# krispy-kenay/WebDGS

Hardware: AMD Instinct MI355X
Metric: training iters/sec (fwd+bwd+Adam), 1M Gaussians @1080p SH3 (higher is better)
Workload: dtype f32

## Files before the change

### webdgs_amd/csrc/common.h

```cpp
#pragma once
#include <hip/hip_runtime.h>

#include <cstdint>
#include <cstdio>
#include <map>
#include <string>
#include <vector>

#include "../../include/webdgs.h"
#include "devmem.h"

typedef uint32_t u32;
typedef int32_t i32;

void wdgs_set_error(const char* fmt, ...);

#define WDGS_CHECK_HIP(expr)                                                                      \
    do {                                                                                          \
        hipError_t _e = (expr);                                                                   \
        if (_e != hipSuccess) {                                                                   \
            wdgs_set_error("%s failed: %s (%s:%d)", #expr, hipGetErrorString(_e), __FILE__, __LINE__); \
            return WDGS_E_HIP;                                                                    \
        }                                                                                         \
    } while (0)

#define WDGS_REQUIRE(cond, code, ...)  \
    do {                               \
        if (!(cond)) {                 \
            wdgs_set_error(__VA_ARGS__); \
            return (code);             \
        }                              \
    } while (0)

#define WDGS_TRY(expr)                 \
    do {                               \
        int _r = (expr);               \
        if (_r != WDGS_OK) return _r;  \
    } while (0)

struct wdgs_device {
    int ordinal = 0;
    hipStream_t stream = nullptr;
    bool own_stream = false;
    hipStream_t lanes[WDGS_MAX_LANES] = {};
    hipEvent_t lane_events[WDGS_MAX_LANES] = {};
    hipEvent_t lane_marks[WDGS_MAX_BATCH_VIEWS] = {};
    int lane = 0;
    hipEvent_t ticket_events[WDGS_TICKET_RING] = {};
    uint64_t ticket_next = 1;
    u32* host_guard = nullptr;
    bool profiling = false;
    bool capturing = false;
    struct Pending { const char* name; hipEvent_t a, b; };
    std::vector<Pending> pending;
    std::vector<hipEvent_t> event_pool;
    struct Total { u32 launches = 0; float ms = 0.f; };
    std::map<std::string, Total> totals;
    std::vector<wdgs_tiled_forward*> forwards;
    std::map<const void*, wdgs_tiled_forward*> range_tables;
    std::vector<wdgs_tiled_forward*> capture_consumes;
    std::vector<void*> dead_command_buffers;
    int num_cus = 256;
    double* ssim_partials = nullptr;
    u32 ssim_partials_count = 0;
};

inline hipError_t wdgs_sync_lanes(wdgs_device* d) {
    for (int l = 1; l < WDGS_MAX_LANES; l++) {
        if (!d->lanes[l]) continue;
        const hipError_t e = hipStreamSynchronize(d->lanes[l]);
        if (e != hipSuccess) return e;
    }
    return hipStreamSynchronize(d->lanes[0] ? d->lanes[0] : d->stream);
}

struct KernelScope {
    wdgs_device* d;
    const char* name;
    hipEvent_t a = nullptr, b = nullptr;
    KernelScope(wdgs_device* dev, const char* n) : d(dev), name(n) {
        if (d->profiling && !d->capturing) {
            a = take(); b = take();
            (void)hipEventRecord(a, d->stream);
        }
    }
    ~KernelScope() {
        if (a) {
            (void)hipEventRecord(b, d->stream);
            d->pending.push_back({name, a, b});
        }
    }
    hipEvent_t take() {
        if (!d->event_pool.empty()) { hipEvent_t e = d->event_pool.back(); d->event_pool.pop_back(); return e; }
        hipEvent_t e; (void)hipEventCreate(&e); return e;
    }
};

#define WDGS_LAUNCH(dev, kname, kernel, grid, block, shmem, ...)                           \
    do {                                                                                   \
        KernelScope _ks((dev), (kname));                                                   \
        hipLaunchKernelGGL(kernel, (grid), (block), (shmem), (dev)->stream, __VA_ARGS__);  \
    } while (0)

constexpr u32 CS_PLANES = 7;
struct CsView {
    float4* planes;
    u32 pitch;
    __device__ __forceinline__ float4& quad(u32 k, u32 idx) const { return planes[(size_t)k * pitch + idx]; }
};

__device__ __forceinline__ u32 xcd_contiguous(u32 b, u32 g) {
    const u32 k = b & 7u, j = b >> 3, q = g >> 3, r = g & 7u;
    return k * q + min(k, r) + j;
}

static inline u32 ceil_div(u32 a, u32 b) { return (a + b - 1u) / b; }
static inline u32 bits_for(u32 v) {
    u32 b = 0;
    while (v) { b++; v >>= 1; }
    return b;
}

constexpr u32 SSIM_WG_PER_CU = 2;
static inline size_t align_up(size_t a, size_t b) { return (a + b - 1) / b * b; }

using wdgs::DevMem;
bool wdgs_device_alive(const wdgs_device* d);

struct RenderSettings { float gaussian_scaling, sh_deg, viewport_x, viewport_y, point_size_px, gaussian_mode, max_splat_radius_px; };
struct TileInfo { u32 num_tiles_x, num_tiles_y, total_tiles, max_tile_entries; };
```

### webdgs_amd/csrc/project.hip

```cpp
#include "launch.h"
#include "wgslm.h"

namespace {

__constant__ float SH_C2c[5] = {1.0925484305920792f, -1.0925484305920792f, 0.31539156525252005f, -1.0925484305920792f, 0.5462742152960396f};
__constant__ float SH_C3c[7] = {-0.5900435899266435f, 2.890611442640554f, -0.4570457994644658f, 0.3731763325901154f,
                                -0.4570457994644658f, 1.445305721320277f, -0.5900435899266435f};

struct ShRow { u32 w[24]; };
WD_DEV ShRow load_sh_row(const u32* __restrict__ sh_buffer, u32 idx, u32 sh_deg) {
    ShRow r;
#pragma unroll
    for (u32 i = 0; i < 24u; i++) r.w[i] = 0u;
    const uint4* q = reinterpret_cast<const uint4*>(sh_buffer + (size_t)idx * 24);
    const u32 nq = (sh_deg == 0u) ? 1u : (sh_deg == 1u) ? 2u : (sh_deg == 2u) ? 4u : 6u;
#pragma unroll
    for (u32 i = 0; i < 6u; i++)
        if (i < nq) { const uint4 v = q[i]; r.w[4 * i] = v.x; r.w[4 * i + 1] = v.y; r.w[4 * i + 2] = v.z; r.w[4 * i + 3] = v.w; }
    return r;
}
WD_DEV float sh_half(const ShRow& sh, u32 h) {
    const u32 w = sh.w[h >> 1];
    return (h & 1u) ? wd_unpack_hi(w) : wd_unpack_lo(w);
}
// ... 241 lines not shown
            if (total > capacity) host_mirror[2] = total;
            host_mirror[3] = 0u;
        }
    }
}

__global__ __launch_bounds__(256) void emit_kernel(u32 n, const u32* __restrict__ splats, const u32* __restrict__ depths,
                                                    const u32* __restrict__ tile_counts, u32* __restrict__ tile_offsets,
                                                    const u32* __restrict__ block_offsets, RenderSettings settings, TileInfo ti,
                                                    u32* __restrict__ keys, u32* __restrict__ values, u32 capacity) {
    __shared__ u32 s_pre[4][64], s_org[4][64], s_w[4][64], s_inv[4][64], s_dep[4][64];
    __shared__ u32 s_wtot[4];
    const u32 idx = blockIdx.x * blockDim.x + threadIdx.x;
    const u32 lane = threadIdx.x & 63u, wave = threadIdx.x >> 6;
    u32 cnt = 0u, org = 0u, width = 1u, depth16 = 0u;
    if (idx < n) {
        const u32 num_tiles = tile_counts[idx];
        if (num_tiles != 0u) {
            const uint2 w01 = *reinterpret_cast<const uint2*>(splats + (size_t)idx * 6);
            const vec2 ndc = V2(wd_unpack_lo(w01.x), wd_unpack_hi(w01.x));
            const float cap = (settings.max_splat_radius_px > 0.0f) ? settings.max_splat_radius_px : 1e9f;
            const vec2 ext = V2(wd_min(wd_unpack_lo(w01.y), cap), wd_min(wd_unpack_hi(w01.y), cap));
            const vec2 viewport = V2(settings.viewport_x, settings.viewport_y);
            const TileBox tb = tile_box(ndc, ext, viewport, ti.num_tiles_x, ti.num_tiles_y, false);
            if (tb.valid) {
                width = tb.max_x - tb.min_x + 1u;
                cnt = width * (tb.max_y - tb.min_y + 1u);
                org = tb.min_y * ti.num_tiles_x + tb.min_x;
                depth16 = depths[idx] >> 16u;
            }
        }
    }
    u32 inc = cnt;
#pragma unroll
    for (u32 d = 1; d < 64; d <<= 1) {
        const u32 t = __shfl_up(inc, d, 64);
        if (lane >= d) inc += t;
    }
    const u32 total = (u32)__shfl((int)inc, 63, 64);
    const u32 wave_first = idx - lane;
    u32 start0;
    if (block_offsets) {
        if (lane == 0u) s_wtot[wave] = total;
        __syncthreads();
        start0 = block_offsets[blockIdx.x];
#pragma unroll
        for (u32 w = 0; w < 4u; w++) start0 += (w < wave) ? s_wtot[w] : 0u;
        if (idx < n) tile_offsets[idx] = start0 + inc - cnt;
        if (total == 0u) return;
    } else {
        if (total == 0u) return;
        start0 = tile_offsets[wave_first];
    }
    s_pre[wave][lane] = inc - cnt;
    s_org[wave][lane] = org;
    s_w[wave][lane] = width;
    s_inv[wave][lane] = 0xFFFFFFFFu / width + 1u;
    s_dep[wave][lane] = depth16;
    __builtin_amdgcn_fence(__ATOMIC_RELEASE, "wavefront");
    __builtin_amdgcn_wave_barrier();
    const u32* pre = s_pre[wave];
    for (u32 e = lane; e < total; e += 64u) {
        u32 o = 0u;
#pragma unroll
        for (u32 step = 32u; step >= 1u; step >>= 1) o += (pre[o + step] <= e) ? step : 0u;
        const u32 k = e - pre[o];
        const u32 w = s_w[wave][o];
        const u32 row = (w == 1u) ? k : __umulhi(k, s_inv[wave][o]);
        const u32 tile_id = s_org[wave][o] + row * ti.num_tiles_x + (k - row * w);
        const u32 key_idx = start0 + e;
        if (key_idx < capacity) {
            keys[key_idx] = ((tile_id + 1u) << 16u) | s_dep[wave][o];
            values[key_idx] = wave_first + o;
        }
    }
}


constexpr u32 ES_CHUNK = 2048;
constexpr u32 ES_ROUNDS = ES_CHUNK / 256;
__global__ __launch_bounds__(256) void emit_scatter_kernel(u32 n, const u32* __restrict__ splats, const u32* __restrict__ depths,
                                                            const u32* __restrict__ tile_counts, u32* __restrict__ tile_offsets,
                                                            const u32* __restrict__ block_offsets, RenderSettings settings, TileInfo ti,
                                                            const u32* __restrict__ column_offsets ,
                                                            const u32* __restrict__ column_totals, u32 inv_ntx ,
                                                            u32* __restrict__ keys, u32* __restrict__ values, u32 capacity) {
    __shared__ u32 s_pre[256];
    __shared__ u32 s_box[256];
    __shared__ u32 s_inv[256], s_dep[256];
    __shared__ u32 whist[4][256];
    __shared__ u32 s_gbase[256];
    __shared__ u32 s_delta[256];
    __shared__ __align__(16) u32 s_keys[ES_CHUNK];
    __shared__ __align__(16) u32 s_vals[ES_CHUNK];
    __shared__ u32 s_wsum[4], s_tsum[4];
    unsigned short* const s_own = reinterpret_cast<unsigned short*>(s_vals);
    const u32 wg = xcd_contiguous(blockIdx.x, gridDim.x);
    const u32 idx = wg * 256u + threadIdx.x;
    const u32 lane = threadIdx.x & 63u, wave = threadIdx.x >> 6;
    const u32 ntx = ti.num_tiles_x;
    u32 cnt = 0u, ox = 0u, oy = 0u, width = 1u, depth16 = 0u;
    const u32 col = threadIdx.x;
    const bool in_range = idx < n;
    const u32 num_tiles = in_range ? tile_counts[idx] : 0u;
    const uint2 w01 = in_range ? *reinterpret_cast<const uint2*>(splats + (size_t)idx * 6) : make_uint2(0u, 0u);
    const u32 depth_all = in_range ? depths[idx] : 0u;
    const u32 tot_c = (col < ntx) ? column_totals[col] : 0u;
    const u32 off_c = (col < ntx) ? column_offsets[(size_t)col * gridDim.x + wg] : 0u;
    const u32 wg_offset = block_offsets[wg];
    if (num_tiles != 0u) {
        const vec2 ndc = V2(wd_unpack_lo(w01.x), wd_unpack_hi(w01.x));
        const float cap = (settings.max_splat_radius_px > 0.0f) ? settings.max_splat_radius_px : 1e9f;
        const vec2 ext = V2(wd_min(wd_unpack_lo(w01.y), cap), wd_min(wd_unpack_hi(w01.y), cap));
        const vec2 viewport = V2(settings.viewport_x, settings.viewport_y);
        const TileBox tb = tile_box(ndc, ext, viewport, ti.num_tiles_x, ti.num_tiles_y, false);
        if (tb.valid) {
            width = tb.max_x - tb.min_x + 1u;
            cnt = width * (tb.max_y - tb.min_y + 1u);
            ox = tb.min_x; oy = tb.min_y;
            depth16 = depth_all >> 16u;
        }
    }
    u32 inc = cnt;
#pragma unroll
    for (u32 d = 1; d < 64; d <<= 1) {
        const u32 t = __shfl_up(inc, d, 64);
        if (lane >= d) inc += t;
    }
    if (lane == 63u) s_wsum[wave] = inc;
    u32 tinc = tot_c;
#pragma unroll
    for (u32 d = 1; d < 64; d <<= 1) {
        const u32 t = __shfl_up(tinc, d, 64);
        if (lane >= d) tinc += t;
    }
    if (lane == 63u) s_tsum[wave] = tinc;
    __syncthreads();
    u32 woff = 0u, total = 0u, tbase = tinc - tot_c;
#pragma unroll
    for (u32 w = 0; w < 4u; w++) {
        const u32 v = s_wsum[w];
        woff += (w < wave) ? v : 0u;
        total += v;
        tbase += (w < wave) ? s_tsum[w] : 0u;
    }
    const u32 pre = woff + inc - cnt;
    if (idx < n) tile_offsets[idx] = wg_offset + pre;
    if (total == 0u) return;
    s_pre[threadIdx.x] = pre;
    s_box[threadIdx.x] = ox | (oy << 8u) | (width << 16u);
    s_inv[threadIdx.x] = 0xFFFFFFFFu / width + 1u;
    s_dep[threadIdx.x] = depth16;
    s_gbase[col] = tbase + off_c;
    const unsigned long long lt_mask = (1ull << lane) - 1ull;
    const u32 wg_first = wg * 256u;
    auto column_of = [&](u32 key) { const u32 t = (key >> 16u) - 1u; return t - __umulhi(t, inv_ntx) * ntx; };
    for (u32 c0 = 0u; c0 < total; c0 += ES_CHUNK) {
        const u32 n_here = min(ES_CHUNK, total - c0);
        const u32 per_wave = ((n_here + 3u) / 4u + 63u) & ~63u;
        const u32 rounds = per_wave / 64u;
#pragma unroll
        for (u32 w = 0; w < 4u; w++) whist[w][threadIdx.x] = 0u;
        reinterpret_cast<uint4*>(s_own)[threadIdx.x] = make_uint4(0u, 0u, 0u, 0u);
        __syncthreads();
        if (cnt != 0u && pre + cnt > c0 && pre < c0 + n_here) s_own[max(pre, c0) - c0] = (unsigned short)(threadIdx.x + 1u);
        __syncthreads();
        {
            const uint4 q = reinterpret_cast<const uint4*>(s_own)[threadIdx.x];
            u32 o[8] = {q.x & 0xFFFFu, q.x >> 16, q.y & 0xFFFFu, q.y >> 16, q.z & 0xFFFFu, q.z >> 16, q.w & 0xFFFFu, q.w >> 16};
#pragma unroll
            for (u32 j = 1; j < 8u; j++) o[j] = max(o[j], o[j - 1u]);
            u32 minc = o[7];
#pragma unroll
            for (u32 d = 1; d < 64; d <<= 1) {
                const u32 t = __shfl_up(minc, d, 64);
                if (lane >= d) minc = max(minc, t);
            }
            if (lane == 63u) s_wsum[wave] = minc;
            __syncthreads();
            u32 carry = __shfl_up(minc, 1, 64);
            if (lane == 0u) carry = 0u;
#pragma unroll
            for (u32 w = 0; w < 4u; w++) carry = max(carry, (w < wave) ? s_wsum[w] : 0u);
#pragma unroll
            for (u32 j = 0; j < 8u; j++) o[j] = max(o[j], carry);
            reinterpret_cast<uint4*>(s_own)[threadIdx.x] = make_uint4(o[0] | (o[1] << 16), o[2] | (o[3] << 16), o[4] | (o[5] << 16), o[6] | (o[7] << 16));
        }
        __syncthreads();
        u32 kk[ES_ROUNDS], vv[ES_ROUNDS], rk[ES_ROUNDS];
#pragma unroll
        for (u32 j = 0; j < ES_ROUNDS; j++) {
            kk[j] = 0xFFFFFFFFu; vv[j] = 0u; rk[j] = 0u;
            if (j < rounds) {
                const u32 i = wave * per_wave + j * 64u + lane;
                const bool valid = i < n_here;
                const u32 o = valid ? (u32)s_own[i] - 1u : 0u;
                const u32 k = c0 + (valid ? i : 0u) - s_pre[o];
                const u32 box = s_box[o];
                const u32 w = box >> 16u;
                const u32 row = (w == 1u) ? k : __umulhi(k, s_inv[o]);
                const u32 cx = (box & 0xFFu) + (k - row * w);
                const u32 tile_id = (((box >> 8u) & 0xFFu) + row) * ntx + cx;
                kk[j] = valid ? (((tile_id + 1u) << 16u) | s_dep[o]) : 0xFFFFFFFFu;
                vv[j] = wg_first + o;
                const u32 digit = valid ? cx : 0u;
                unsigned long long m = __ballot(valid);
#pragma unroll
                for (u32 b = 0; b < 8; b++) {
                    const bool bit = (digit >> b) & 1u;
                    const unsigned long long bal = __ballot(bit);
                    m &= bit ? bal : ~bal;
                }
                const u32 pre_c = whist[wave][digit];
                const u32 below = (u32)__popcll(m & lt_mask);
                rk[j] = pre_c + below;
                if (valid && below == 0u) whist[wave][digit] = pre_c + (u32)__popcll(m);
            }
        }
        __syncthreads();
        {
            u32 cnt_c = 0u;
#pragma unroll
            for (u32 w = 0; w < 4u; w++) cnt_c += whist[w][col];
            u32 cinc = cnt_c;
#pragma unroll
            for (u32 d = 1; d < 64; d <<= 1) {
                const u32 t = __shfl_up(cinc, d, 64);
                if (lane >= d) cinc += t;
            }
            if (lane == 63u) s_wsum[wave] = cinc;
            __syncthreads();
            u32 lstart = cinc - cnt_c;
#pragma unroll
            for (u32 w = 0; w < 4u; w++) lstart += (w < wave) ? s_wsum[w] : 0u;
            const u32 gb = s_gbase[col];
            s_delta[col] = gb - lstart;
            s_gbase[col] = gb + cnt_c;
            u32 run = lstart;
#pragma unroll
            for (u32 w = 0; w < 4u; w++) {
                const u32 c = whist[w][col];
                whist[w][col] = run;
                run += c;
            }
        }
        __syncthreads();
#pragma unroll
        for (u32 j = 0; j < ES_ROUNDS; j++) {
            if (j < rounds) {
                const u32 i = wave * per_wave + j * 64u + lane;
                if (i < n_here) {
                    const u32 lpos = whist[wave][column_of(kk[j])] + rk[j];
                    s_keys[lpos] = kk[j];
                    s_vals[lpos] = vv[j];
                }
            }
        }
        __syncthreads();
        for (u32 e = threadIdx.x; e < n_here; e += 256u) {
            const u32 key = s_keys[e];
            const u32 pos = s_delta[column_of(key)] + e;
            if (pos < capacity) {
                keys[pos] = key;
                values[pos] = s_vals[e];
            }
        }
        __syncthreads();
    }
}

}

int launch_project_count(wdgs_device* dev, u32 n, const u32* gaussians, const u32* sh, const float* camera, const RenderSettings& st, const TileInfo& ti, u32* splats,
                         u32* depths, u32* counts, u32* visible_shards, u32* block_counts, u32* column_counts, const u32* dc_words, u32* nf_stamp, const u32* nf_frame) {
    if (n == 0) return WDGS_OK;
    WDGS_LAUNCH(dev, "project_count", project_count_kernel, dim3(ceil_div(n, 256)), dim3(256), 0, n, gaussians, sh, camera, st, ti, splats, depths, counts, visible_shards,
                block_counts, column_counts, dc_words, nf_stamp, nf_frame);
    WDGS_CHECK_HIP(hipGetLastError());
    return WDGS_OK;
}

int launch_project_count_views(wdgs_device* dev, u32 n, const u32* gaussians, const u32* sh, const RenderSettings& st, const TileInfo& ti, const ProjectViews& pv,
                               const u32* dc_words) {
    if (n == 0 || pv.count == 0) return WDGS_OK;
    WDGS_LAUNCH(dev, "project_count_views", project_count_views_kernel, dim3(ceil_div(n, 256)), dim3(256), 0, n, gaussians, sh, st, ti, pv, dc_words);
    WDGS_CHECK_HIP(hipGetLastError());
    return WDGS_OK;
}

int launch_update_stats(wdgs_device* dev, u32 n, const u32* offsets, const u32* counts, u32 capacity, u32* stats, u32* visible_shards, u32* host_mirror) {
    WDGS_LAUNCH(dev, "update_stats", update_stats_kernel, dim3(1), dim3(64), 0, n, offsets, counts, capacity, stats, visible_shards, host_mirror);
    WDGS_CHECK_HIP(hipGetLastError());
    return WDGS_OK;
}

int launch_emit_scatter(wdgs_device* dev, u32 n, const u32* splats, const u32* depths, const u32* counts, u32* offsets, const u32* block_offsets,
                        const RenderSettings& st, const TileInfo& ti, const u32* column_offsets, const u32* column_totals, u32* keys, u32* values, u32 capacity) {
    if (n == 0) return WDGS_OK;
    WDGS_LAUNCH(dev, "emit_scatter", emit_scatter_kernel, dim3(ceil_div(n, 256)), dim3(256), 0, n, splats, depths, counts, offsets, block_offsets, st, ti, column_offsets,
                column_totals, 0xFFFFFFFFu / ti.num_tiles_x + 1u , keys, values, capacity);
    WDGS_CHECK_HIP(hipGetLastError());
    return WDGS_OK;
}

int launch_emit(wdgs_device* dev, u32 n, const u32* splats, const u32* depths, const u32* counts, u32* offsets, const u32* block_offsets, const RenderSettings& st,
                const TileInfo& ti, u32* keys, u32* values, u32 capacity) {
    if (n == 0) return WDGS_OK;
    WDGS_LAUNCH(dev, "emit", emit_kernel, dim3(ceil_div(n, 256)), dim3(256), 0, n, splats, depths, counts, offsets, block_offsets, st, ti, keys, values, capacity);
    WDGS_CHECK_HIP(hipGetLastError());
    return WDGS_OK;
}
```

### webdgs_amd/csrc/sort.hip

```cpp
#include <algorithm>
#include <memory>

#include "launch.h"
#include "longlist.h"

namespace {

constexpr u32 SORT_THREADS = 256;
constexpr u32 SORT_ITEMS_MAX = 16;
constexpr u32 SORT_TILE_MAX = SORT_THREADS * SORT_ITEMS_MAX;
constexpr u32 RADIX = 256;

struct DigitOf {
    u32 shift, dmask, row_inv;
    __device__ __forceinline__ u32 operator()(u32 key) const { return row_inv ? min(__umulhi((key >> 16u) - 1u, row_inv), dmask) : ((key >> shift) & dmask); }
};

template <u32 ITEMS>
__global__ __launch_bounds__(SORT_THREADS) void sort_hist_kernel(const u32* __restrict__ keys, const u32* __restrict__ count_ptr, DigitOf digit_of,
                                                                 u32 num_parts, u32* __restrict__ counts , u32* __restrict__ ranges_init,
                                                                 u32 total_tiles, u32* __restrict__ marks_init) {
    constexpr u32 TILE = SORT_THREADS * ITEMS;
    __shared__ u32 lh[SORT_THREADS / 64][RADIX];
    const u32 count = *count_ptr;
    const u32 part = blockIdx.x;
    const u32 base = part * TILE;
    const u32 dmask = digit_of.dmask;
    if (ranges_init) {
        const u32 active = max((count + TILE - 1u) / TILE, 1u);
        if (part < active)
            for (u32 t = part * SORT_THREADS + threadIdx.x; t <= total_tiles; t += active * SORT_THREADS) ranges_init[t] = (t == total_tiles) ? count : 0xFFFFFFFFu;
    }
    if (marks_init) {
        const u32 active = max((count + TILE - 1u) / TILE, 1u);
        if (part < active)
            for (u32 t = part * SORT_THREADS + threadIdx.x; t < total_tiles; t += active * SORT_THREADS) marks_init[t] = 0u;
    }
    if (base >= count) return;
    const u32 wave = threadIdx.x >> 6;
#pragma unroll
    for (u32 w = 0; w < SORT_THREADS / 64; w++) lh[w][threadIdx.x] = 0;
    __syncthreads();
    if (base + TILE <= count) {
#pragma unroll
        for (u32 j = 0; j < ITEMS / 4; j++) {
            const uint4 q = *reinterpret_cast<const uint4*>(keys + base + (j * SORT_THREADS + threadIdx.x) * 4u);
            const u32 d0 = digit_of(q.x), d1 = digit_of(q.y), d2 = digit_of(q.z), d3 = digit_of(q.w);
            if (d0 == d3 && d0 == d1 && d0 == d2) {
                atomicAdd(&lh[wave][d0], 4u);
            } else {
                atomicAdd(&lh[wave][d0], 1u);
                atomicAdd(&lh[wave][d1], 1u);
                atomicAdd(&lh[wave][d2], 1u);
                atomicAdd(&lh[wave][d3], 1u);
            }
        }
    } else {
        for (u32 j = 0; j < ITEMS; j++) {
            const u32 i = base + j * SORT_THREADS + threadIdx.x;
            if (i < count) atomicAdd(&lh[wave][digit_of(keys[i])], 1u);
        }
    }
    __syncthreads();
    if (threadIdx.x <= dmask) counts[(size_t)threadIdx.x * num_parts + part] = lh[0][threadIdx.x] + lh[1][threadIdx.x] + lh[2][threadIdx.x] + lh[3][threadIdx.x];
}

template <u32 ITEMS>
__global__ __launch_bounds__(256) void sort_scan_rows_kernel(u32* __restrict__ counts, const u32* __restrict__ count_ptr, u32 num_parts,
                                                              u32* __restrict__ totals) {
    constexpr u32 TILE = SORT_THREADS * ITEMS;
    __shared__ u32 s_w[4];
    const u32 active = (*count_ptr + TILE - 1u) / TILE;
    u32* row = counts + (size_t)blockIdx.x * num_parts;
    const u32 lane = threadIdx.x & 63u, wave = threadIdx.x >> 6;
    u32 carry = 0;
    for (u32 base = 0; base < active; base += 1024u) {
        const u32 i0 = base + threadIdx.x * 4u;
        u32 x[4];
#pragma unroll
        for (u32 j = 0; j < 4; j++) x[j] = (i0 + j < active) ? row[i0 + j] : 0u;
        const u32 tsum = x[0] + x[1] + x[2] + x[3];
        u32 inc = tsum;
#pragma unroll
        for (u32 d = 1; d < 64; d <<= 1) {
            const u32 t = __shfl_up(inc, d, 64);
            if (lane >= d) inc += t;
        }
        if (lane == 63u) s_w[wave] = inc;
        __syncthreads();
        u32 woff = 0, tot = 0;
#pragma unroll
        for (u32 w = 0; w < 4; w++) { const u32 v = s_w[w]; if (w < wave) woff += v; tot += v; }
        __syncthreads();
        u32 run = carry + woff + inc - tsum;
#pragma unroll
        for (u32 j = 0; j < 4; j++) {
            if (i0 + j < active) row[i0 + j] = run;
            run += x[j];
        }
        carry += tot;
    }
    if (threadIdx.x == 0) totals[blockIdx.x] = carry;
}

template <u32 ITEMS>
__global__ __launch_bounds__(SORT_THREADS) void sort_scatter_kernel(const u32* __restrict__ keys_in, const u32* __restrict__ vals_in,
                                                                    u32* __restrict__ keys_out, u32* __restrict__ vals_out,
                                                                    const u32* __restrict__ count_ptr, DigitOf digit_of, u32 num_parts,
                                                                    const u32* __restrict__ offsets , const u32* __restrict__ digit_totals,
                                                                    u32* __restrict__ ranges, u32 ranges_mode, u32 total_tiles) {
    constexpr u32 TILE = SORT_THREADS * ITEMS;
    __shared__ u32 whist[SORT_THREADS / 64][RADIX];
    const u32 dmask = digit_of.dmask;
    const u32 count = *count_ptr;
    const u32 active_parts = max((count + TILE - 1u) / TILE, 1u);
    if (blockIdx.x >= active_parts) return;
    const u32 part = xcd_contiguous(blockIdx.x, active_parts);
    const u32 base = part * TILE;
    if (ranges_mode == 1u) {
        const u32 active = max((count + TILE - 1u) / TILE, 1u);
        if (part < active)
            for (u32 t = part * SORT_THREADS + threadIdx.x; t <= total_tiles; t += active * SORT_THREADS) ranges[t] = (t == total_tiles) ? count : 0xFFFFFFFFu;
    }
    if (base >= count) return;
    const u32 lane = threadIdx.x & 63u, wave = threadIdx.x >> 6;
    const u32 tot_d_early = (threadIdx.x <= dmask) ? digit_totals[threadIdx.x] : 0u;
    const u32 off_d_early = (threadIdx.x <= dmask) ? offsets[(size_t)threadIdx.x * num_parts + part] : 0u;
#pragma unroll
    for (u32 w = 0; w < SORT_THREADS / 64; w++) whist[w][threadIdx.x] = 0;
    __syncthreads();

    u32 k[ITEMS], v[ITEMS], rk[ITEMS];
    const unsigned long long lt_mask = (1ull << lane) - 1ull;
#pragma unroll
    for (u32 j = 0; j < ITEMS; j++) {
        const u32 i = base + wave * (ITEMS * 64u) + j * 64u + lane;
        const bool valid = i < count;
        k[j] = valid ? keys_in[i] : 0xFFFFFFFFu;
        v[j] = valid ? vals_in[i] : 0u;
    }
#pragma unroll
    for (u32 j = 0; j < ITEMS; j++) {
        const u32 i = base + wave * (ITEMS * 64u) + j * 64u + lane;
        const bool valid = i < count;
        const u32 digit = valid ? digit_of(k[j]) : 0u;
        unsigned long long m = __ballot(valid);
#pragma unroll
        for (u32 b = 0; b < 8; b++) {
            const bool bit = (digit >> b) & 1u;
            const unsigned long long bal = __ballot(bit);
            m &= bit ? bal : ~bal;
        }
        const u32 pre = whist[wave][digit];
        const u32 below = (u32)__popcll(m & lt_mask);
        rk[j] = pre + below;
        if (valid && below == 0u) whist[wave][digit] = pre + (u32)__popcll(m);
    }
    __syncthreads();
    __shared__ u32 s_keys[TILE];
    __shared__ u32 s_vals[TILE];
    __shared__ u32 s_gdelta[RADIX];
    __shared__ u32 s_wsum[SORT_THREADS / 64];
    {
        const u32 d = threadIdx.x;
        u32 cnt_d = 0;
#pragma unroll
        for (u32 w = 0; w < SORT_THREADS / 64; w++) cnt_d += whist[w][d];
        u32 inc = cnt_d;
#pragma unroll
        for (u32 s = 1; s < 64; s <<= 1) {
            const u32 t = __shfl_up(inc, s, 64);
            if (lane >= s) inc += t;
        }
        if (lane == 63u) s_wsum[wave] = inc;
        __syncthreads();
        u32 woff = 0;
#pragma unroll
        for (u32 w = 0; w < SORT_THREADS / 64; w++) if (w < wave) woff += s_wsum[w];
        const u32 local_start = woff + inc - cnt_d;
        const u32 tot_d = tot_d_early;
        u32 tinc = tot_d;
#pragma unroll
        for (u32 s = 1; s < 64; s <<= 1) {
            const u32 t = __shfl_up(tinc, s, 64);
            if (lane >= s) tinc += t;
        }
        __syncthreads();
        if (lane == 63u) s_wsum[wave] = tinc;
        __syncthreads();
        u32 tbase = tinc - tot_d;
#pragma unroll
        for (u32 w = 0; w < SORT_THREADS / 64; w++) if (w < wave) tbase += s_wsum[w];
        s_gdelta[d] = tbase + off_d_early - local_start;
        u32 run = local_start;
#pragma unroll
        for (u32 w = 0; w < SORT_THREADS / 64; w++) {
            const u32 c = whist[w][d];
            whist[w][d] = run;
            run += c;
        }
    }
    __syncthreads();
#pragma unroll
    for (u32 j = 0; j < ITEMS; j++) {
        const u32 i = base + wave * (ITEMS * 64u) + j * 64u + lane;
        if (i < count) {
            const u32 digit = digit_of(k[j]);
            const u32 lpos = whist[wave][digit] + rk[j];
            s_keys[lpos] = k[j];
            s_vals[lpos] = v[j];
        }
    }
    __syncthreads();
    const u32 n_here = min(TILE, count - base);
#pragma unroll 4
    for (u32 e = threadIdx.x; e < n_here; e += SORT_THREADS) {
        const u32 key = s_keys[e];
        const u32 pos = s_gdelta[digit_of(key)] + e;
        keys_out[pos] = key;
        vals_out[pos] = s_vals[e];
        if (ranges_mode == 2u && (e == 0u || (s_keys[e - 1u] >> 16u) != (key >> 16u)) && (key >> 16u) - 1u < total_tiles) atomicMin(&ranges[(key >> 16u) - 1u], pos);
    }
}

__global__ __launch_bounds__(256) void tile_ranges_kernel(const u32* __restrict__ keys, const u32* __restrict__ count_ptr, u32 total_tiles,
                                                           u32* __restrict__ ranges) {
    const u32 t = blockIdx.x * 4u + (threadIdx.x >> 6);
    const u32 lane = threadIdx.x & 63u;
    if (t > total_tiles) return;
    const u32 count = *count_ptr;
    if (t == total_tiles) { if (lane == 0u) ranges[t] = count; return; }
    const u32 want = t + 1u;
    u32 lo = 0u, hi = count;
    while (hi - lo > 64u) {
        const u32 span = hi - lo;
        const u32 pos = lo + (u32)(((unsigned long long)span * (lane + 1u)) / 65ull);
        const bool less = (keys[pos] >> 16u) < want;
        const unsigned long long m = __ballot(less);
        const u32 k = (u32)__popcll(m);
        const u32 pos_prev = (k == 0u) ? lo : lo + (u32)(((unsigned long long)span * k) / 65ull) + 1u;
        const u32 pos_next = (k == 64u) ? hi : lo + (u32)(((unsigned long long)span * (k + 1u)) / 65ull);
        lo = pos_prev;
        hi = pos_next;
    }
    const u32 idx = lo + lane;
    const bool ge = idx < hi && (keys[idx] >> 16u) >= want;
    const unsigned long long m = __ballot(ge);
    const u32 first = (m == 0ull) ? hi : lo + (u32)__builtin_ctzll(m);
    if (lane == 0u) ranges[t] = (first < count && (keys[first] >> 16u) == want) ? first : 0xFFFFFFFFu;
}

constexpr u32 SEG_CAP = 2048;
constexpr u32 SEG_THREADS = 256;

constexpr u32 SEG_ROUNDS = SEG_CAP / SEG_THREADS;
constexpr u32 SEG_WIDE_BITS = 10;
constexpr u32 SEG_BINS = 1u << SEG_WIDE_BITS;
typedef unsigned short seg_hist_t;
template <u32 BITS>
__device__ __forceinline__ void seg_pass_regs(const u32 (&kk)[SEG_ROUNDS], const u32 (&vv)[SEG_ROUNDS], u32* __restrict__ dst_k, u32* __restrict__ dst_v, u32 n,
                                              u32 per_wave, u32 sub, u32 shift, seg_hist_t (*whist)[SEG_BINS], u32* s_wsum) {
    constexpr u32 BINS = 1u << BITS, PER_THREAD = BINS / SEG_THREADS;
    static_assert(BINS <= SEG_BINS && BINS % SEG_THREADS == 0, "digit width");
    const u32 lane = threadIdx.x & 63u, wave = threadIdx.x >> 6;
    const u32 rounds = per_wave / 64u;
    const unsigned long long lt_mask = (1ull << lane) - 1ull;
    auto digit_of = [&](u32 key) { return (((key & 0xFFFFu) - sub) >> shift) & (BINS - 1u); };
#pragma unroll
    for (u32 w = 0; w < SEG_THREADS / 64; w++)
#pragma unroll
        for (u32 j = 0; j < PER_THREAD; j++) whist[w][threadIdx.x * PER_THREAD + j] = 0;
    __syncthreads();
    u32 rk[SEG_ROUNDS];
#pragma unroll
    for (u32 j = 0; j < SEG_ROUNDS; j++) {
        if (j < rounds) {
            const u32 i = wave * per_wave + j * 64u + lane;
            const bool valid = i < n;
            const u32 digit = digit_of(kk[j]);
            unsigned long long m = __ballot(valid);
#pragma unroll
            for (u32 b = 0; b < BITS; b++) {
                const bool bit = (digit >> b) & 1u;
                const unsigned long long bal = __ballot(bit);
                m &= bit ? bal : ~bal;
            }
            const u32 pre = whist[wave][digit];
            const u32 below = (u32)__popcll(m & lt_mask);
            rk[j] = pre + below;
            if (valid && below == 0u) whist[wave][digit] = (seg_hist_t)(pre + (u32)__popcll(m));
        }
    }
    __syncthreads();
    {
        u32 cnt[PER_THREAD], tsum = 0;
#pragma unroll
        for (u32 j = 0; j < PER_THREAD; j++) {
            const u32 d = threadIdx.x * PER_THREAD + j;
            cnt[j] = 0;
#pragma unroll
            for (u32 w = 0; w < SEG_THREADS / 64; w++) cnt[j] += whist[w][d];
            tsum += cnt[j];
        }
        u32 inc = tsum;
#pragma unroll
        for (u32 sft = 1; sft < 64; sft <<= 1) {
            const u32 t = __shfl_up(inc, sft, 64);
            if (lane >= sft) inc += t;
        }
        if (lane == 63u) s_wsum[wave] = inc;
        __syncthreads();
        u32 run = inc - tsum;
#pragma unroll
        for (u32 w = 0; w < SEG_THREADS / 64; w++) if (w < wave) run += s_wsum[w];
#pragma unroll
        for (u32 j = 0; j < PER_THREAD; j++) {
            const u32 d = threadIdx.x * PER_THREAD + j;
#pragma unroll
            for (u32 w = 0; w < SEG_THREADS / 64; w++) {
                const u32 c = whist[w][d];
                whist[w][d] = (seg_hist_t)run;
                run += c;
            }
        }
    }
    __syncthreads();
#pragma unroll
    for (u32 j = 0; j < SEG_ROUNDS; j++) {
        if (j < rounds) {
            const u32 i = wave * per_wave + j * 64u + lane;
            if (i < n) {
                const u32 pos = (u32)whist[wave][digit_of(kk[j])] + rk[j];
                dst_k[pos] = kk[j];
                dst_v[pos] = vv[j];
            }
        }
    }
    __syncthreads();
}

WD_DEV void lds_barrier() { asm volatile("s_waitcnt lgkmcnt(0)\n\ts_barrier" ::: "memory"); }

__device__ void seg_pass_global(const u32* __restrict__ src_k, const u32* __restrict__ src_v, u32* __restrict__ dst_k, u32* __restrict__ dst_v, u32 n,
                                u32 shift, seg_hist_t (*whist)[SEG_BINS], u32* s_base , u32* s_wsum) {
    const u32 lane = threadIdx.x & 63u, wave = threadIdx.x >> 6;
    const unsigned long long lt_mask = (1ull << lane) - 1ull;
    s_base[threadIdx.x] = 0u;
    __syncthreads();
    for (u32 i0 = threadIdx.x; i0 < n; i0 += 4u * SEG_THREADS) {
        u32 kh[4];
#pragma unroll
        for (u32 j = 0; j < 4; j++) kh[j] = (i0 + j * SEG_THREADS < n) ? src_k[i0 + j * SEG_THREADS] : 0u;
#pragma unroll
        for (u32 j = 0; j < 4; j++)
            if (i0 + j * SEG_THREADS < n) atomicAdd(&s_base[(kh[j] >> shift) & (RADIX - 1u)], 1u);
    }
    __syncthreads();
    {
        const u32 cnt_d = s_base[threadIdx.x];
        u32 inc = cnt_d;
#pragma unroll
        for (u32 sft = 1; sft < 64; sft <<= 1) {
            const u32 t = __shfl_up(inc, sft, 64);
            if (lane >= sft) inc += t;
        }
        if (lane == 63u) s_wsum[wave] = inc;
        __syncthreads();
        u32 woff = 0;
#pragma unroll
        for (u32 w = 0; w < SEG_THREADS / 64; w++) if (w < wave) woff += s_wsum[w];
        s_base[threadIdx.x] = woff + inc - cnt_d;
    }
    __syncthreads();
    seg_hist_t* const cnt16 = &whist[0][0];
    uint4* const my_counts = reinterpret_cast<uint4*>(cnt16 + threadIdx.x * 16u);
    u32 kq[4], vq[4];
#pragma unroll
    for (u32 j = 0; j < 4u; j++) {
        const u32 i = j * SEG_THREADS + threadIdx.x;
        kq[j] = (i < n) ? src_k[i] : 0xFFFFFFFFu;
        vq[j] = (i < n) ? src_v[i] : 0u;
    }
    for (u32 c0 = 0; c0 < n; c0 += 4u * SEG_THREADS) {
        u32 kn[4], vn[4];
#pragma unroll
        for (u32 j = 0; j < 4u; j++) {
            const u32 i_next = c0 + (4u + j) * SEG_THREADS + threadIdx.x;
            kn[j] = (i_next < n) ? src_k[i_next] : 0xFFFFFFFFu;
            vn[j] = (i_next < n) ? src_v[i_next] : 0u;
        }
        my_counts[0] = make_uint4(0u, 0u, 0u, 0u);
        my_counts[1] = make_uint4(0u, 0u, 0u, 0u);
        u32 below[4], group[4];
#pragma unroll
        for (u32 j = 0; j < 4u; j++) {
            const bool valid = c0 + j * SEG_THREADS + threadIdx.x < n;
            const u32 digit = (kq[j] >> shift) & (RADIX - 1u);
            unsigned long long m = __ballot(valid);
#pragma unroll
            for (u32 b = 0; b < 8; b++) {
                const bool bit = (digit >> b) & 1u;
                const unsigned long long bal = __ballot(bit);
                m &= bit ? bal : ~bal;
            }
            below[j] = (u32)__popcll(m & lt_mask);
            group[j] = (valid && below[j] == 0u) ? (u32)__popcll(m) : 0u;
        }
        lds_barrier();
#pragma unroll
        for (u32 j = 0; j < 4u; j++)
            if (group[j] != 0u) cnt16[((kq[j] >> shift) & (RADIX - 1u)) * 16u + j * 4u + wave] = (seg_hist_t)group[j];
        lds_barrier();
        u32 trip_total = 0u;
        {
            uint4 q[2] = {my_counts[0], my_counts[1]};
            u32* const w = reinterpret_cast<u32*>(q);
#pragma unroll
            for (u32 x = 0; x < 8u; x++) {
                const u32 lo = w[x] & 0xFFFFu, hi = w[x] >> 16u;
                w[x] = trip_total | ((trip_total + lo) << 16u);
                trip_total += lo + hi;
            }
            my_counts[0] = q[0];
            my_counts[1] = q[1];
        }
        lds_barrier();
#pragma unroll
        for (u32 j = 0; j < 4u; j++) {
            if (c0 + j * SEG_THREADS + threadIdx.x < n) {
                const u32 digit = (kq[j] >> shift) & (RADIX - 1u);
                const u32 pos = s_base[digit] + cnt16[digit * 16u + j * 4u + wave] + below[j];
                dst_k[pos] = kq[j];
                dst_v[pos] = vq[j];
            }
        }
        lds_barrier();
        s_base[threadIdx.x] += trip_total;
#pragma unroll
        for (u32 j = 0; j < 4u; j++) { kq[j] = kn[j]; vq[j] = vn[j]; }
    }
    __syncthreads();
}

__device__ void long_list_build(const LongWork& lw, u32 t, u32 n) {
    __shared__ u32 s_first, s_lb;
    const bool want = lw.threshold != 0u && n > lw.threshold && !(lw.nf_stamp && lw.nf_stamp[t] == *lw.nf_frame);
    if (!want) return;
    const u32 chunks = (n + 63u) >> 6, need = 4u * chunks;
    if (threadIdx.x == 0u) {
        s_first = atomicAdd(&lw.hdr[LL_ITEMS], need);
        s_lb = atomicAdd(&lw.hdr[LL_BLOCKS], 4u);
    }
    __syncthreads();
    const u32 first = s_first, lb = s_lb;
    const bool items_fit = first + need <= lw.max_items && first + need >= first, blocks_fit = lb + 4u <= lw.max_blocks;
    const bool ok = items_fit && blocks_fit;
    for (u32 i = threadIdx.x; i < need && first + i < lw.max_items && first + i >= first; i += SEG_THREADS) lw.item_block[first + i] = ok ? lb + i / chunks : 0xFFFFFFFFu;
    if (threadIdx.x < 4u && lb + threadIdx.x < lw.max_blocks) {
        const u32 b = lb + threadIdx.x;
        lw.blocks[b] = LongBlock{t, threadIdx.x, first + threadIdx.x * chunks, ok ? chunks : 0u};
        lw.sync[b] = LongSync{0u, LL_NO_ROWS, 0u, 0u, 0u, 0u, 0u, 0u};
    }
    if (threadIdx.x == 0u && ok) lw.flags[t] = 0xFu;
}

__global__ __launch_bounds__(SEG_THREADS, 6) void segment_sort_kernel(u32* __restrict__ cur_k, u32* __restrict__ cur_v, u32* __restrict__ alt_k,
                                                                    u32* __restrict__ alt_v, const u32* __restrict__ ranges, u32 total_tiles, LongWork lw) {
    __shared__ u32 a_k[SEG_CAP], a_v[SEG_CAP];
    __shared__ seg_hist_t whist[SEG_THREADS / 64][SEG_BINS];
    __shared__ u32 s_base[RADIX];
    __shared__ u32 s_wsum[SEG_THREADS / 64];
    __shared__ u32 s_min[SEG_THREADS / 64], s_max[SEG_THREADS / 64];
    const u32 t = blockIdx.x;
    const u32 start = ranges[t];
    u32 end = ranges[t + 1u];
    if (start == 0xFFFFFFFFu) return;
    for (u32 nx = t + 1u; end == 0xFFFFFFFFu && nx < total_tiles;) { nx++; end = ranges[nx]; }
    if (lw.flags) long_list_build(lw, t, (end != 0xFFFFFFFFu && end > start) ? end - start : 0u);
    if (end <= start + 1u || end == 0xFFFFFFFFu) return;
    const u32 n = end - start;
    if (n <= SEG_CAP) {
        const u32 lane = threadIdx.x & 63u, wave = threadIdx.x >> 6;
        const u32 per_wave = ((n + 3u) / 4u + 63u) & ~63u;
        const u32 rounds = per_wave / 64u;
        u32 kk[SEG_ROUNDS], vv[SEG_ROUNDS];
#pragma unroll
        for (u32 j = 0; j < SEG_ROUNDS; j++) {
            const u32 i = wave * per_wave + j * 64u + lane;
            const bool valid = j < rounds && i < n;
            kk[j] = valid ? cur_k[start + i] : 0xFFFFFFFFu;
            vv[j] = valid ? cur_v[start + i] : 0u;
        }
        u32 lo16 = 0xFFFFu, hi16 = 0u;
#pragma unroll
        for (u32 j = 0; j < SEG_ROUNDS; j++) {
            const u32 i = wave * per_wave + j * 64u + lane;
            if (j < rounds && i < n) { lo16 = min(lo16, kk[j] & 0xFFFFu); hi16 = max(hi16, kk[j] & 0xFFFFu); }
        }
#pragma unroll
        for (u32 d = 32; d >= 1; d >>= 1) {
            lo16 = min(lo16, (u32)__shfl_xor((int)lo16, (int)d, 64));
            hi16 = max(hi16, (u32)__shfl_xor((int)hi16, (int)d, 64));
        }
        if (lane == 0u) { s_min[wave] = lo16; s_max[wave] = hi16; }
        __syncthreads();
        lo16 = min(min(s_min[0], s_min[1]), min(s_min[2], s_min[3]));
        hi16 = max(max(s_max[0], s_max[1]), max(s_max[2], s_max[3]));
        if (hi16 - lo16 < (1u << 8)) {
            seg_pass_regs<8>(kk, vv, a_k, a_v, n, per_wave, lo16, 0u, whist, s_wsum);
        } else if (hi16 - lo16 < (1u << 9)) {
            seg_pass_regs<9>(kk, vv, a_k, a_v, n, per_wave, lo16, 0u, whist, s_wsum);
        } else if (hi16 - lo16 < SEG_BINS) {
            seg_pass_regs<SEG_WIDE_BITS>(kk, vv, a_k, a_v, n, per_wave, lo16, 0u, whist, s_wsum);
        } else {
            seg_pass_regs<8>(kk, vv, a_k, a_v, n, per_wave, 0u, 0u, whist, s_wsum);
#pragma unroll
            for (u32 j = 0; j < SEG_ROUNDS; j++) {
                const u32 i = wave * per_wave + j * 64u + lane;
                const bool valid = j < rounds && i < n;
                kk[j] = valid ? a_k[i] : 0xFFFFFFFFu;
                vv[j] = valid ? a_v[i] : 0u;
            }
            __syncthreads();
            seg_pass_regs<8>(kk, vv, a_k, a_v, n, per_wave, 0u, 8u, whist, s_wsum);
        }
        for (u32 i = threadIdx.x; i < n; i += SEG_THREADS) { cur_k[start + i] = a_k[i]; cur_v[start + i] = a_v[i]; }
    } else {
        seg_pass_global(cur_k + start, cur_v + start, alt_k + start, alt_v + start, n, 0u, whist, s_base, s_wsum);
        __syncthreads();
        seg_pass_global(alt_k + start, alt_v + start, cur_k + start, cur_v + start, n, 8u, whist, s_base, s_wsum);
    }
}

}

struct wdgs_sorter {
    wdgs_device* dev = nullptr;
    u32 capacity = 0;
    u32 items = 0;
    u32 num_parts = 0;
    const u32* count_ptr = nullptr;
    DevMem<u32> keys[2];
    DevMem<u32> vals[2];
    DevMem<u32> counts;
    DevMem<u32> totals;
    int final_out_index = 0;
};

extern "C" {

int wdgs_sorter_create(wdgs_device* dev, uint32_t max_capacity, const void* stats_dev, wdgs_sorter** out) {
    WDGS_REQUIRE(dev && out && stats_dev, WDGS_E_INVALID, "wdgs_sorter_create: null argument");
    WDGS_REQUIRE(max_capacity <= 0xFFFFF000u, WDGS_E_CAPACITY, "sorter capacity %u too large", max_capacity);
    auto s = std::make_unique<wdgs_sorter>();
    s->dev = dev;
    s->capacity = (u32)align_up(max_capacity > 0 ? max_capacity : 1, SORT_TILE_MAX);
    s->items = s->capacity <= (8u << 20) ? 4u : SORT_ITEMS_MAX;
    s->num_parts = s->capacity / (SORT_THREADS * s->items);
// ... 157 lines not shown
```

Baseline: 1277.

## Streamline wave digit matching and halve LDS staging in radix scatter

Result: faster. 1294, median of 6 (+1.4%).

```diff
diff --git a/webdgs_amd/csrc/common.h b/webdgs_amd/csrc/common.h
--- a/webdgs_amd/csrc/common.h
+++ b/webdgs_amd/csrc/common.h
@@ -114,6 +114,21 @@
     return k * q + min(k, r) + j;
 }
 
+template <u32 BITS>
+__device__ __forceinline__ unsigned long long match_digit(u32 digit, unsigned long long among) {
+    u32 lo = (u32)among, hi = (u32)(among >> 32);
+#pragma unroll
+    for (u32 b = 0; b < BITS; b++) {
+        const bool bit = (digit & (1u << b)) != 0u;
+        const unsigned long long bal = __builtin_amdgcn_ballot_w64(bit);
+        const u32 x = bit ? 0xFFFFFFFFu : 0u;
+        lo &= ~((u32)bal ^ x);
+        hi &= ~((u32)(bal >> 32) ^ x);
+    }
+    return ((unsigned long long)hi << 32) | lo;
+}
+__device__ __forceinline__ u32 lanes_below(unsigned long long m) { return __builtin_amdgcn_mbcnt_hi((u32)(m >> 32), __builtin_amdgcn_mbcnt_lo((u32)m, 0u)); }
+
 static inline u32 ceil_div(u32 a, u32 b) { return (a + b - 1u) / b; }
 static inline u32 bits_for(u32 v) {
     u32 b = 0;
diff --git a/webdgs_amd/csrc/project.hip b/webdgs_amd/csrc/project.hip
--- a/webdgs_amd/csrc/project.hip
+++ b/webdgs_amd/csrc/project.hip
@@ -417,7 +417,6 @@
     s_inv[threadIdx.x] = 0xFFFFFFFFu / width + 1u;
     s_dep[threadIdx.x] = depth16;
     s_gbase[col] = tbase + off_c;
-    const unsigned long long lt_mask = (1ull << lane) - 1ull;
     const u32 wg_first = wg * 256u;
     auto column_of = [&](u32 key) { const u32 t = (key >> 16u) - 1u; return t - __umulhi(t, inv_ntx) * ntx; };
     for (u32 c0 = 0u; c0 < total; c0 += ES_CHUNK) {
@@ -469,15 +468,9 @@
                 kk[j] = valid ? (((tile_id + 1u) << 16u) | s_dep[o]) : 0xFFFFFFFFu;
                 vv[j] = wg_first + o;
                 const u32 digit = valid ? cx : 0u;
-                unsigned long long m = __ballot(valid);
-#pragma unroll
-                for (u32 b = 0; b < 8; b++) {
-                    const bool bit = (digit >> b) & 1u;
-                    const unsigned long long bal = __ballot(bit);
-                    m &= bit ? bal : ~bal;
-                }
+                const unsigned long long m = match_digit<8>(digit, __ballot(valid));
                 const u32 pre_c = whist[wave][digit];
-                const u32 below = (u32)__popcll(m & lt_mask);
+                const u32 below = lanes_below(m);
                 rk[j] = pre_c + below;
                 if (valid && below == 0u) whist[wave][digit] = pre_c + (u32)__popcll(m);
             }
diff --git a/webdgs_amd/csrc/sort.hip b/webdgs_amd/csrc/sort.hip
--- a/webdgs_amd/csrc/sort.hip
+++ b/webdgs_amd/csrc/sort.hip
@@ -130,8 +130,7 @@
     for (u32 w = 0; w < SORT_THREADS / 64; w++) whist[w][threadIdx.x] = 0;
     __syncthreads();
 
-    u32 k[ITEMS], v[ITEMS], rk[ITEMS];
-    const unsigned long long lt_mask = (1ull << lane) - 1ull;
+    u32 k[ITEMS], v[ITEMS], rk2[ITEMS / 2];
 #pragma unroll
     for (u32 j = 0; j < ITEMS; j++) {
         const u32 i = base + wave * (ITEMS * 64u) + j * 64u + lane;
@@ -144,21 +143,15 @@
         const u32 i = base + wave * (ITEMS * 64u) + j * 64u + lane;
         const bool valid = i < count;
         const u32 digit = valid ? digit_of(k[j]) : 0u;
-        unsigned long long m = __ballot(valid);
-#pragma unroll
-        for (u32 b = 0; b < 8; b++) {
-            const bool bit = (digit >> b) & 1u;
-            const unsigned long long bal = __ballot(bit);
-            m &= bit ? bal : ~bal;
-        }
+        const unsigned long long m = match_digit<8>(digit, __ballot(valid));
         const u32 pre = whist[wave][digit];
-        const u32 below = (u32)__popcll(m & lt_mask);
-        rk[j] = pre + below;
+        const u32 below = lanes_below(m);
+        rk2[j / 2u] = (j & 1u) ? (rk2[j / 2u] | ((pre + below) << 16u)) : (pre + below);
+        asm volatile("" : "+v"(rk2[j / 2u]));
         if (valid && below == 0u) whist[wave][digit] = pre + (u32)__popcll(m);
     }
     __syncthreads();
-    __shared__ u32 s_keys[TILE];
-    __shared__ u32 s_vals[TILE];
+    __shared__ u32 s_stage[TILE];
     __shared__ u32 s_gdelta[RADIX];
     __shared__ u32 s_wsum[SORT_THREADS / 64];
     {
@@ -206,20 +199,37 @@
         const u32 i = base + wave * (ITEMS * 64u) + j * 64u + lane;
         if (i < count) {
             const u32 digit = digit_of(k[j]);
-            const u32 lpos = whist[wave][digit] + rk[j];
-            s_keys[lpos] = k[j];
-            s_vals[lpos] = v[j];
+            const u32 lpos = whist[wave][digit] + ((rk2[j / 2u] >> ((j & 1u) * 16u)) & 0xFFFFu);
+            s_stage[lpos] = k[j];
+            rk2[j / 2u] = (j & 1u) ? ((rk2[j / 2u] & 0xFFFFu) | (lpos << 16u)) : ((rk2[j / 2u] & 0xFFFF0000u) | lpos);
         }
     }
     __syncthreads();
     const u32 n_here = min(TILE, count - base);
-#pragma unroll 4
-    for (u32 e = threadIdx.x; e < n_here; e += SORT_THREADS) {
-        const u32 key = s_keys[e];
-        const u32 pos = s_gdelta[digit_of(key)] + e;
+    u32 dg4[ITEMS / 4];
+#pragma unroll
+    for (u32 r = 0; r < ITEMS; r++) {
+        const u32 e = r * SORT_THREADS + threadIdx.x;
+        if ((r & 3u) == 0u) dg4[r / 4u] = 0u;
+        if (e >= n_here) continue;
+        const u32 key = s_stage[e];
+        const u32 digit = digit_of(key);
+        const u32 pos = s_gdelta[digit] + e;
+        dg4[r / 4u] |= digit << ((r & 3u) * 8u);
         keys_out[pos] = key;
-        vals_out[pos] = s_vals[e];
-        if (ranges_mode == 2u && (e == 0u || (s_keys[e - 1u] >> 16u) != (key >> 16u)) && (key >> 16u) - 1u < total_tiles) atomicMin(&ranges[(key >> 16u) - 1u], pos);
+        if (ranges_mode == 2u && (e == 0u || (s_stage[e - 1u] >> 16u) != (key >> 16u)) && (key >> 16u) - 1u < total_tiles) atomicMin(&ranges[(key >> 16u) - 1u], pos);
+    }
+    __syncthreads();
+#pragma unroll
+    for (u32 j = 0; j < ITEMS; j++) {
+        const u32 i = base + wave * (ITEMS * 64u) + j * 64u + lane;
+        if (i < count) s_stage[(rk2[j / 2u] >> ((j & 1u) * 16u)) & 0xFFFFu] = v[j];
+    }
+    __syncthreads();
+#pragma unroll
+    for (u32 r = 0; r < ITEMS; r++) {
+        const u32 e = r * SORT_THREADS + threadIdx.x;
+        if (e < n_here) vals_out[s_gdelta[(dg4[r / 4u] >> ((r & 3u) * 8u)) & 0xFFu] + e] = s_stage[e];
     }
 }
 
@@ -264,7 +274,6 @@
     static_assert(BINS <= SEG_BINS && BINS % SEG_THREADS == 0, "digit width");
     const u32 lane = threadIdx.x & 63u, wave = threadIdx.x >> 6;
     const u32 rounds = per_wave / 64u;
-    const unsigned long long lt_mask = (1ull << lane) - 1ull;
     auto digit_of = [&](u32 key) { return (((key & 0xFFFFu) - sub) >> shift) & (BINS - 1u); };
 #pragma unroll
     for (u32 w = 0; w < SEG_THREADS / 64; w++)
@@ -278,15 +287,9 @@
             const u32 i = wave * per_wave + j * 64u + lane;
             const bool valid = i < n;
             const u32 digit = digit_of(kk[j]);
-            unsigned long long m = __ballot(valid);
-#pragma unroll
-            for (u32 b = 0; b < BITS; b++) {
-                const bool bit = (digit >> b) & 1u;
-                const unsigned long long bal = __ballot(bit);
-                m &= bit ? bal : ~bal;
-            }
+            const unsigned long long m = match_digit<BITS>(digit, __ballot(valid));
             const u32 pre = whist[wave][digit];
-            const u32 below = (u32)__popcll(m & lt_mask);
+            const u32 below = lanes_below(m);
             rk[j] = pre + below;
             if (valid && below == 0u) whist[wave][digit] = (seg_hist_t)(pre + (u32)__popcll(m));
         }
@@ -344,7 +347,6 @@
 __device__ void seg_pass_global(const u32* __restrict__ src_k, const u32* __restrict__ src_v, u32* __restrict__ dst_k, u32* __restrict__ dst_v, u32 n,
                                 u32 shift, seg_hist_t (*whist)[SEG_BINS], u32* s_base , u32* s_wsum) {
     const u32 lane = threadIdx.x & 63u, wave = threadIdx.x >> 6;
-    const unsigned long long lt_mask = (1ull << lane) - 1ull;
     s_base[threadIdx.x] = 0u;
     __syncthreads();
     for (u32 i0 = threadIdx.x; i0 < n; i0 += 4u * SEG_THREADS) {
@@ -396,14 +398,8 @@
         for (u32 j = 0; j < 4u; j++) {
             const bool valid = c0 + j * SEG_THREADS + threadIdx.x < n;
             const u32 digit = (kq[j] >> shift) & (RADIX - 1u);
-            unsigned long long m = __ballot(valid);
-#pragma unroll
-            for (u32 b = 0; b < 8; b++) {
-                const bool bit = (digit >> b) & 1u;
-                const unsigned long long bal = __ballot(bit);
-                m &= bit ? bal : ~bal;
-            }
-            below[j] = (u32)__popcll(m & lt_mask);
+            const unsigned long long m = match_digit<8>(digit, __ballot(valid));
+            below[j] = lanes_below(m);
             group[j] = (valid && below[j] == 0u) ? (u32)__popcll(m) : 0u;
         }
         lds_barrier();
```
